# snimu/mixture-of-tokenizers

Measured on AMD Instinct MI355X. Metric: mixed-embed tokens/sec at BxT=256x2048; achieved HBM GB/s vs peak, higher is better.
Workload: dtype f32

## Files before the change

### mixture-of-tokenizers_amd/csrc/mot_embed.hip

```cpp
#include <stdlib.h>

#include <algorithm>

#include "mot_wave.hpp"

namespace mot {

template <int MODE, int NCH, int U, typename T, bool DUAL>
struct MixStream {
    typedef typename Elem<T>::vec vec_t;
    typedef typename Elem<T>::raw raw_t;
    static constexpr int VEC = Elem<T>::kVec;
    const MixArgs &A;
    const WaveLds &W;
    const T *tok_table, *byte_table;
    int lane, Dm, nchunk, ntok;
    int tokv = 0, unit_lane0 = 0;
    bool act[NCH];
    bool tact[NCH];
    raw_t ar[U][NCH];

    __device__ __forceinline__ MixStream(const MixArgs &A_, const WaveLds &W_, int ntok_) : A(A_), W(W_), ntok(ntok_) {
        tok_table = (const T *)A.tok_table;
        byte_table = (const T *)A.byte_table;
// ... 185 lines not shown
#endif
    };
    if (has_ids && A.id_source == MOT_IDS_FROM_TTB) {
        if (A.ttb_elem == 2) {
            if (A.pull_dir == kPullLeft) from_ttb(WaveIndexer<kPullLeft, int16_t>(A, W, row, u0, ntok, dual));
            else if (A.pull_dir == kPullRight) from_ttb(WaveIndexer<kPullRight, int16_t>(A, W, row, u0, ntok, dual));
            else from_ttb(WaveIndexer<kPullNone, int16_t>(A, W, row, u0, ntok, dual));
        } else {
            if (A.pull_dir == kPullLeft) from_ttb(WaveIndexer<kPullLeft, int32_t>(A, W, row, u0, ntok, dual));
            else if (A.pull_dir == kPullRight) from_ttb(WaveIndexer<kPullRight, int32_t>(A, W, row, u0, ntok, dual));
            else from_ttb(WaveIndexer<kPullNone, int32_t>(A, W, row, u0, ntok, dual));
        }
    } else {
        S.tokv = lane < ntok ? A.tokens[row * A.T + u0 + lane] : 0;
        S.request(0);
        if (has_ids) wave_ids_given(A, W, row, u0, ntok);
        else if (A.counters && lane == 0) atomicAdd((unsigned long long *)A.counters, (unsigned long long)ntok);
    }

    T *orow = (T *)A.out + (row * A.T + u0) * (int64_t)S.Dm;
    S.run([&](int t) { return orow + (int64_t)t * S.Dm; });
}

constexpr int kRouteUnits = 8;
constexpr int64_t kRouteMinTokens = 131072;
constexpr int kClaimShards = 64;
constexpr int kClaimStride = 64;

struct RouteWs {
    uint32_t *claim;
    uint8_t *ends;
    uint8_t *offs;
    uint16_t *ids;
    uint16_t *ids2;
};

template <int DIR, typename E>
__global__ __launch_bounds__(kThreads) void route_index_kernel(const MixArgs A, const RouteWs R) {
    extern __shared__ __attribute__((aligned(16))) unsigned char lds_wave[];
    const int lane = threadIdx.x & 63;
    const int wave = __builtin_amdgcn_readfirstlane(threadIdx.x >> 6);
    if (blockIdx.x < 2) R.claim[(blockIdx.x * kThreads + threadIdx.x) * kClaimStride] = 0;
    const int64_t unit_id = (int64_t)blockIdx.x * kWaves + wave;
    if (unit_id >= A.n_units) return;
    const int64_t row = unit_id / A.units_per_row;
    const int64_t u0 = (unit_id - row * A.units_per_row) * A.unit;
    const int ntok = (int)min((int64_t)A.unit, A.T - u0);
    const bool dual = A.add_padded != 0;
    const WaveLds W = wave_lds_carve(lds_wave + (size_t)wave * A.wave_lds, A.unit, A.bpt, dual, DIR != kPullNone ? A.ttb_elem : 0);
    WaveIndexer<DIR, E> ix(A, W, row, u0, ntok, dual);
    const int tok = ix.tokens();
    ix.load_rows();
    ix.finish();

    const int bpt = A.bpt, sv = bpt | 1, n = ntok * bpt;
    const int64_t base = (row * A.T + u0) * bpt;
    for (int i = lane; i < n; i += 64) {
        const int t = i / bpt, k = i - t * bpt;
        R.ids[base + i] = (uint16_t)W.ids[t * sv + k];
        if (dual) R.ids2[base + i] = (uint16_t)W.ids2[t * sv + k];
    }
    const bool in = ix.in_unit;
    const int b = tok & 7;
    int rank = 0, end = 0, acc = 0;
#pragma unroll
    for (int q = 0; q < 8; ++q) {
        const unsigned long long m = __ballot(in && b == q);
        if (in && b == q) rank = acc + (int)__builtin_amdgcn_mbcnt_hi((unsigned)(m >> 32), __builtin_amdgcn_mbcnt_lo((unsigned)m, 0u));
        acc += __popcll(m);
        if (lane == q) end = acc;
    }
    if (in) R.offs[unit_id * A.unit + rank] = (uint8_t)ix.j;
    if (lane < 8) R.ends[unit_id * 8 + lane] = (uint8_t)end;
}

template <int NCH, int U, typename T, bool DUAL>
__global__ __launch_bounds__(kThreads) void embed_mix_routed_kernel(const MixArgs A, const RouteWs R) {
    extern __shared__ __attribute__((aligned(16))) unsigned char lds_wave[];
    const int lane = threadIdx.x & 63;
    const int wave = __builtin_amdgcn_readfirstlane(threadIdx.x >> 6);
    const WaveLds W = wave_lds_carve(lds_wave + (size_t)wave * A.wave_lds, 64, A.bpt, DUAL, 0);
    MixStream<MOT_MIX_SUM, NCH, U, T, DUAL> S(A, W, 0);
    const int bpt = A.bpt, sv = bpt | 1;
    const int64_t n_chunks = (A.n_units + kRouteUnits - 1) / kRouteUnits;
    const int home = blockIdx.x & 7;
    const int shard = ((blockIdx.x >> 3) * kWaves + wave) % kClaimShards;
    for (int q = 0; q < 8;) {
        const int b = (home + q) & 7;
        const int64_t lo = n_chunks * shard / kClaimShards, hi = n_chunks * (shard + 1) / kClaimShards;
        uint32_t k = 0;
        if (lane == 0) k = atomicAdd(R.claim + (b * kClaimShards + shard) * kClaimStride, 1u);
        const int64_t c = lo + __builtin_amdgcn_readfirstlane(k);
        if (c >= hi) { ++q; continue; }
        const int64_t uc = c * kRouteUnits;
        int nb = 0, sb = 0;
        if (lane < kRouteUnits && uc + lane < A.n_units) {
            const uint8_t *e = R.ends + (uc + lane) * 8;
            sb = b ? e[b - 1] : 0;
            nb = e[b] - sb;
        }
        const int incl = wave_scan_add(nb), excl = incl - nb;
        const int total = __builtin_amdgcn_readlane(incl, kRouteUnits - 1);
        for (int p0 = 0; p0 < total; p0 += 64) {
            const int l = p0 + lane;
            int g = 0;
#pragma unroll
            for (int gg = 1; gg < kRouteUnits; ++gg) g = l >= __builtin_amdgcn_readlane(excl, gg) ? gg : g;
            const int ex = __shfl(excl, g, 64), st = __shfl(sb, g, 64);
            int64_t pos = 0;
            int tok = 0;
            if (l < total) {
                const int64_t u = uc + g;
                const int64_t row = u / A.units_per_row;
                pos = row * A.T + (u - row * A.units_per_row) * A.unit + R.offs[u * A.unit + st + (l - ex)];
                tok = A.tokens[pos];
                if ((uint64_t)(uint32_t)tok >= (uint64_t)A.ttb_rows) tok = 0;
            }
            S.tokv = tok;
            S.ntok = min(64, total - p0);
            S.request(0);
            if (l < total) {
                const uint16_t *ia = R.ids + pos * bpt, *ib = R.ids2 + pos * bpt;
                if ((bpt & 7) == 0) {
                    typedef uint16_t u16x8 __attribute__((ext_vector_type(8)));
                    for (int k = 0; k < bpt; k += 8) {
                        const u16x8 va = *(const u16x8 *)(ia + k);
                        u16x8 vb;
                        if (DUAL) vb = *(const u16x8 *)(ib + k);
#pragma unroll
                        for (int e = 0; e < 8; ++e) {
                            W.ids[lane * sv + k + e] = va[e];
                            if (DUAL) W.ids2[lane * sv + k + e] = vb[e];
                        }
                    }
                } else {
                    for (int k = 0; k < bpt; ++k) {
                        W.ids[lane * sv + k] = ia[k];
                        if (DUAL) W.ids2[lane * sv + k] = ib[k];
                    }
                }
            }
            wave_lds_sync();
            const int plo = (int)(uint32_t)pos, phi = (int)(pos >> 32);
            S.run([&](int t) {
                const int64_t p = (int64_t)(((uint64_t)(uint32_t)__builtin_amdgcn_readlane(phi, t) << 32) |
                                            (uint32_t)__builtin_amdgcn_readlane(plo, t));
                return (T *)A.out + p * (int64_t)S.Dm;
            });
            wave_lds_sync();
        }
    }
}

template <typename T>
__global__ __launch_bounds__(kThreads) void rows_rnorm_kernel(const T *__restrict__ table, int64_t rows, int dim,
                                                              float eps, float *__restrict__ out) {
    const int lane = threadIdx.x & 63;
    const int64_t r = (int64_t)blockIdx.x * kWaves + (threadIdx.x >> 6);
    if (r >= rows) return;
    float ss = 0.f;
    for (int j = lane; j < dim; j += 64) {
        const float v = Elem<T>::load1(table + r * dim + j);
        ss += v * v;
    }
    ss = wave_sum(ss);
    if (lane == 0) out[r] = rms_scale(ss, dim, eps);
}

template <int G, typename IdT, typename T>
__global__ __launch_bounds__(kThreads) void gather_rows_kernel(const IdT *__restrict__ ids_a, const IdT *__restrict__ ids_b,
                                                               int64_t n, const T *__restrict__ table, int64_t rows,
                                                               int dim, int rms, float eps, const float *scale,
                                                               T *__restrict__ out, uint32_t *status, int group, int64_t out_ld,
                                                               uint32_t oor_flag) {
// ... 143 lines not shown
                       uint32_t *status, int dtype, hipStream_t stream) {
    if (n == 0) return MOT_OK;
    const unsigned blocks = (unsigned)((n + kWaves - 1) / kWaves);
    if (dtype == MOT_BF16)
        hipLaunchKernelGGL(concat_rows_kernel<__bf16>, dim3(blocks), dim3(kThreads), 0, stream, tokens, ids, n, (const __bf16 *)tok_table, tok_rows, Dt,
                           (const __bf16 *)byte_table, byte_rows, Db, bpt, norm_tok, byte_rnorm, eps, (__bf16 *)u, K, tok_lo, byte_lo, status);
    else
        hipLaunchKernelGGL(concat_rows_kernel<float>, dim3(blocks), dim3(kThreads), 0, stream, tokens, ids, n, (const float *)tok_table, tok_rows, Dt,
                           (const float *)byte_table, byte_rows, Db, bpt, norm_tok, byte_rnorm, eps, (float *)u, K, tok_lo, byte_lo, status);
    return check_launch("concat_rows_kernel");
}

int launch_rows_rnorm(const void *table, int64_t rows, int dim, float eps, float *out, int dtype, hipStream_t stream) {
    const int64_t rb = (rows + kWaves - 1) / kWaves;
    if (dtype == MOT_BF16)
        hipLaunchKernelGGL(rows_rnorm_kernel<__bf16>, dim3((unsigned)rb), dim3(kThreads), 0, stream, (const __bf16 *)table, rows, dim, eps, out);
    else
        hipLaunchKernelGGL(rows_rnorm_kernel<float>, dim3((unsigned)rb), dim3(kThreads), 0, stream, (const float *)table, rows, dim, eps, out);
    return check_launch("rows_rnorm_kernel");
}

static int pick_unit(int64_t n_tokens) { return n_tokens >= 131072 ? 32 : 16; }

static bool sum_routed(const MotEmbedMixDesc &d) {
    return d.mode == MOT_MIX_SUM && d.id_source == MOT_IDS_FROM_TTB && !d.out_ids_padded && !d.out_ids_pulled && d.bpt > 0 &&
           d.byte_rows <= 65536 && d.n_rows * d.tokens_per_row >= kRouteMinTokens && d.dtype == MOT_F32 &&
           (uint64_t)d.tok_rows * d.tok_dim * sizeof(float) <= ((uint64_t)256 << 20);
}

struct MixWorkspace {
    size_t rnorm, claim, ends, offs, ids, ids2, total;
};
static MixWorkspace mix_workspace(const MotEmbedMixDesc &d) {
    auto up = [](size_t x) { return (x + 255) & ~(size_t)255; };
    MixWorkspace w{};
    w.total = (d.mode != MOT_MIX_NOOP && d.norm_byte) ? up((size_t)d.byte_rows * sizeof(float)) : 0;
    if (!sum_routed(d)) return w;
    const int64_t tokens = d.n_rows * d.tokens_per_row;
    const int unit = pick_unit(tokens);
    const int64_t n_units = d.n_rows * ((d.tokens_per_row + unit - 1) / unit);
    const size_t id_bytes = up((size_t)tokens * d.bpt * sizeof(uint16_t));
    w.claim = w.total;
    w.ends = w.claim + (size_t)8 * kClaimShards * kClaimStride * sizeof(uint32_t);
    w.offs = w.ends + up((size_t)n_units * 8);
    w.ids = w.offs + up((size_t)n_units * unit);
    w.ids2 = w.ids + id_bytes;
    w.total = w.ids2 + (d.add_padded ? id_bytes : 0);
    return w;
}

size_t embed_mix_workspace_bytes(const MotEmbedMixDesc &d) {
    if (d.mode == MOT_MIX_CONCAT_LINEAR) return d.dtype == MOT_BF16 ? embed_mix_linear_bf16_workspace_bytes(d) : embed_mix_linear_workspace_bytes(d);
    return mix_workspace(d).total;
}

template <int DIR, typename E>
static void launch_route_index(const MixArgs &A, const RouteWs &R, int64_t blocks, size_t lds, hipStream_t stream) {
    hipLaunchKernelGGL((route_index_kernel<DIR, E>), dim3((unsigned)blocks), dim3(kThreads), lds, stream, A, R);
}

template <int NCH, int U, typename T, bool DUAL>
static int launch_routed(const MixArgs &A, const RouteWs &R, int64_t blocks, size_t lds, hipStream_t stream) {
    if (A.ttb_elem == 2) {
        if (A.pull_dir == kPullLeft) launch_route_index<kPullLeft, int16_t>(A, R, blocks, lds, stream);
        else if (A.pull_dir == kPullRight) launch_route_index<kPullRight, int16_t>(A, R, blocks, lds, stream);
        else launch_route_index<kPullNone, int16_t>(A, R, blocks, lds, stream);
    } else {
        if (A.pull_dir == kPullLeft) launch_route_index<kPullLeft, int32_t>(A, R, blocks, lds, stream);
        else if (A.pull_dir == kPullRight) launch_route_index<kPullRight, int32_t>(A, R, blocks, lds, stream);
        else launch_route_index<kPullNone, int32_t>(A, R, blocks, lds, stream);
    }
    if (int rc = check_launch("route_index_kernel")) return rc;
    MixArgs Ar = A;
    Ar.wave_lds = (int)wave_lds_bytes(64, A.bpt, DUAL, 0);
    const size_t lds_r = (size_t)Ar.wave_lds * kWaves;
    const void *kern = (const void *)embed_mix_routed_kernel<NCH, U, T, DUAL>;
    int dev = 0, cus = 0, per_cu = 0;
    if (hipGetDevice(&dev) != hipSuccess || hipDeviceGetAttribute(&cus, hipDeviceAttributeMultiprocessorCount, dev) != hipSuccess ||
        hipOccupancyMaxActiveBlocksPerMultiprocessor(&per_cu, kern, kThreads, lds_r) != hipSuccess || per_cu < 1)
        return set_error(MOT_EHIP, "embed_mix: no occupancy for embed_mix_routed_kernel");
    const int64_t grid = std::max<int64_t>(((int64_t)cus * per_cu) & ~(int64_t)7, 8 * kClaimShards / kWaves);
    hipLaunchKernelGGL((embed_mix_routed_kernel<NCH, U, T, DUAL>), dim3((unsigned)grid), dim3(kThreads), lds_r, stream, Ar, R);
    return check_launch("embed_mix_routed_kernel");
}

template <int MODE, int NCH, int U, typename T>
static int launch_mix(const MixArgs &A, int64_t blocks, size_t lds, hipStream_t stream, const RouteWs *route) {
    const bool dual = MODE != MOT_MIX_NOOP && (A.id_source == MOT_IDS_FROM_TTB ? A.add_padded != 0 : A.ids_b != nullptr);
    if constexpr (MODE == MOT_MIX_SUM && sizeof(T) == 4) {
        if (route) return dual ? launch_routed<NCH, U, T, true>(A, *route, blocks, lds, stream) : launch_routed<NCH, U, T, false>(A, *route, blocks, lds, stream);
    }
    if (dual)
        hipLaunchKernelGGL((embed_mix_kernel<MODE, NCH, U, T, true>), dim3((unsigned)blocks), dim3(kThreads), lds, stream, A);
    else
        hipLaunchKernelGGL((embed_mix_kernel<MODE, NCH, U, T, false>), dim3((unsigned)blocks), dim3(kThreads), lds, stream, A);
    return check_launch("embed_mix_kernel");
}

template <int MODE>
static int dispatch_nch(const MixArgs &A, int dtype, int64_t blocks, size_t lds, hipStream_t stream, const RouteWs *route = nullptr) {
    const int Dm = MODE == MOT_MIX_CONCAT ? A.Dt + A.bpt * A.Db : A.Dt;
    if (dtype == MOT_BF16) {
        switch ((Dm / 8 + 63) / 64) {
            case 1: return launch_mix<MODE, 1, 4, __bf16>(A, blocks, lds, stream, route);
            case 2: return launch_mix<MODE, 2, 4, __bf16>(A, blocks, lds, stream, route);
            case 3: return launch_mix<MODE, 3, 2, __bf16>(A, blocks, lds, stream, route);
            case 4: return launch_mix<MODE, 4, 2, __bf16>(A, blocks, lds, stream, route);
            default: return set_error(MOT_EUNSUPPORTED, "embed_mix: model_dim %d > 2048 is not built", Dm);
        }
    }
    switch ((Dm / 4 + 63) / 64) {
        case 1: return launch_mix<MODE, 1, 4, float>(A, blocks, lds, stream, route);
        case 2: return launch_mix<MODE, 2, 4, float>(A, blocks, lds, stream, route);
        case 3: return launch_mix<MODE, 3, 2, float>(A, blocks, lds, stream, route);
        case 4: return launch_mix<MODE, 4, 2, float>(A, blocks, lds, stream, route);
        case 5:
        case 6: return launch_mix<MODE, 6, 1, float>(A, blocks, lds, stream, route);
        case 7:
        case 8: return launch_mix<MODE, 8, 1, float>(A, blocks, lds, stream, route);
        default: return set_error(MOT_EUNSUPPORTED, "embed_mix: model_dim %d > 2048 is not built", Dm);
    }
}


template <typename T, int U, int BPT, bool NORMB, int ADD = 0>
__global__ __launch_bounds__(1024) void embed_mean_lds_kernel(const MixArgs A, int slice_cols, int nslices, int64_t tokens_per_part) {
    extern __shared__ __attribute__((aligned(16))) unsigned char lds_raw[];
    T *tab = (T *)lds_raw;
    constexpr int VEC = Elem<T>::kVec;
    typedef typename Elem<T>::vec vec_t;
    const int tid = threadIdx.x, lane = tid & 63, wave = tid >> 6;
    const int slice = blockIdx.x % nslices;
    const int64_t part = blockIdx.x / nslices;
    const int col0 = slice * slice_cols;
    const int D = A.Dt;
    const T *byte_table = (const T *)A.byte_table, *tok_table = (const T *)A.tok_table;
    const int pieces_per_row = slice_cols / VEC;
    for (int64_t q = tid; q < A.byte_rows * pieces_per_row; q += 1024) {
        const int r = (int)(q / pieces_per_row), c = (int)(q - (int64_t)r * pieces_per_row) * VEC;
        *(typename Elem<T>::raw *)(tab + (size_t)r * slice_cols + c) = Elem<T>::load_raw(byte_table + (int64_t)r * D + col0 + c);
    }
    __syncthreads();
// ... 185 lines not shown
    A.units_per_row = (d.tokens_per_row + A.unit - 1) / A.unit;
    A.n_units = d.n_rows * A.units_per_row;
    const int64_t blocks = (A.n_units + kWaves - 1) / kWaves;
    if (blocks > 0x7fffffffLL) return set_error(MOT_EUNSUPPORTED, "embed_mix: too many units");
    const int stream_eb = (has_ids && d.id_source == MOT_IDS_FROM_TTB && d.pull_dir != MOT_PULL_NONE) ? d.ttb_elem_bytes : 0;
    A.wave_lds = (int)wave_lds_bytes(A.unit, has_ids ? d.bpt : 0, dual, stream_eb);
    const size_t lds = (size_t)A.wave_lds * kWaves;

    const MixWorkspace ws = mix_workspace(d);
    if (ws.total && (!d.workspace || d.workspace_bytes < ws.total))
        return set_error(MOT_EWORKSPACE, "embed_mix: needs %zu workspace bytes, got %zu", ws.total, d.workspace_bytes);
    if (d.mode != MOT_MIX_NOOP && d.norm_byte) {
        float *rn = (float *)((unsigned char *)d.workspace + ws.rnorm);
        int rc = launch_rows_rnorm(d.byte_table, d.byte_rows, d.byte_dim, A.eps, rn, d.dtype, stream);
        if (rc) return rc;
        A.byte_rnorm = rn;
    }
    if (const int sc = mean_lds_slice(d)) {
        return d.dtype == MOT_BF16 ? launch_mean_lds<__bf16>(A, d, sc, stream) : launch_mean_lds<float>(A, d, sc, stream);
    }
    switch (d.mode) {
        case MOT_MIX_NOOP: return dispatch_nch<MOT_MIX_NOOP>(A, d.dtype, blocks, lds, stream);
        case MOT_MIX_SUM: {
            if (sum_routed(d) && A.unit == pick_unit(d.n_rows * d.tokens_per_row)) {
                unsigned char *w = (unsigned char *)d.workspace;
                const RouteWs R{(uint32_t *)(w + ws.claim), w + ws.ends, w + ws.offs, (uint16_t *)(w + ws.ids), (uint16_t *)(w + ws.ids2)};
                return dispatch_nch<MOT_MIX_SUM>(A, d.dtype, blocks, lds, stream, &R);
            }
            return dispatch_nch<MOT_MIX_SUM>(A, d.dtype, blocks, lds, stream);
        }
        case MOT_MIX_MEAN: return dispatch_nch<MOT_MIX_MEAN>(A, d.dtype, blocks, lds, stream);
        case MOT_MIX_CONCAT: return dispatch_nch<MOT_MIX_CONCAT>(A, d.dtype, blocks, lds, stream);
        default: return set_error(MOT_EINVAL, "embed_mix: bad mode %d", d.mode);
    }
}

}
```

### mixture-of-tokenizers_amd/csrc/mot_group.hip

```cpp
#include "mot_mix.hpp"

namespace mot {

constexpr int kRankThreads = 512;
__device__ __forceinline__ int lower_bound_u32(const uint32_t *a, int n, uint32_t v) {
    int lo = 0, hi = n;
    while (lo < hi) {
        const int mid = (lo + hi) >> 1;
        if (a[mid] < v) lo = mid + 1; else hi = mid;
    }
    return lo;
}
__global__ __launch_bounds__(kThreads) void zero_i32_kernel(int32_t *__restrict__ p, int64_t n) {
    for (int64_t i = (int64_t)blockIdx.x * kThreads + threadIdx.x; i < n; i += (int64_t)gridDim.x * kThreads) p[i] = 0;
}

int launch_zero_words(void *p, int64_t n_words, hipStream_t stream) {
    if (n_words <= 0) return MOT_OK;
    int64_t blocks = (n_words + kThreads - 1) / kThreads;
    if (blocks > 2048) blocks = 2048;
    hipLaunchKernelGGL(zero_i32_kernel, dim3((unsigned)blocks), dim3(kThreads), 0, stream, (int32_t *)p, n_words);
    return check_launch("zero_i32_kernel");
}

template <int kRankChunk>
__global__ __launch_bounds__(kRankThreads) void bwd_rank_kernel(const int32_t *__restrict__ tokens, int64_t n, int64_t rows,
                                                                int32_t *__restrict__ counts, int32_t *__restrict__ rank,
                                                                uint32_t *status) {
    __shared__ uint32_t skey[kRankChunk];
    __shared__ int32_t runbase[kRankChunk];
    const int tid = threadIdx.x;
    const int64_t base = (int64_t)blockIdx.x * kRankChunk;
    for (int i = tid; i < kRankChunk; i += kRankThreads) {
        uint32_t key = 0xffffffffu;
        if (base + i < n) {
            uint32_t t = (uint32_t)tokens[base + i];
            if ((uint64_t)t >= (uint64_t)rows) { if (status) atomicOr(status, kStatusTokenOor); t = 0; }
            key = (t << 11) | (uint32_t)i;
        }
        skey[i] = key;
    }
    __syncthreads();
    for (int k = 2; k <= kRankChunk; k <<= 1)
        for (int j = k >> 1; j > 0; j >>= 1) {
            for (int p = tid; p < kRankChunk / 2; p += kRankThreads) {
                const int i = ((p & ~(j - 1)) << 1) | (p & (j - 1)), ixj = i | j;
                const uint32_t x = skey[i], y = skey[ixj];
                if ((x > y) == ((i & k) == 0)) { skey[i] = y; skey[ixj] = x; }
            }
            __syncthreads();
        }
    constexpr int kPer = kRankChunk / kRankThreads;
    int head[kPer];
#pragma unroll
    for (int r = 0; r < kPer; ++r) {
        const int si = tid + r * kRankThreads;
        const uint32_t key = skey[si];
        head[r] = -1;
        if (key == 0xffffffffu) continue;
        const uint32_t tok = key >> 11;
        const int h = (si == 0 || (skey[si - 1] >> 11) != tok) ? si : lower_bound_u32(skey, si, tok << 11);
        head[r] = h;
        if (h == si) {
            const int e = lower_bound_u32(skey, kRankChunk, (tok + 1) << 11);
            runbase[si] = atomicAdd(&counts[tok], e - si);
        }
    }
    __syncthreads();
#pragma unroll
    for (int r = 0; r < kPer; ++r) {
        const int si = tid + r * kRankThreads;
        if (head[r] < 0) continue;
        rank[base + (skey[si] & 2047)] = runbase[head[r]] + (si - head[r]);
    }
}

__global__ __launch_bounds__(kThreads) void bwd_place_kernel(const int32_t *__restrict__ tokens, int64_t n, int64_t rows,
                                                             const int32_t *__restrict__ starts, const int32_t *__restrict__ rank,
                                                             int32_t *__restrict__ pos_sorted, int32_t *__restrict__ tok_sorted) {
    for (int64_t i = (int64_t)blockIdx.x * kThreads + threadIdx.x; i < n; i += (int64_t)gridDim.x * kThreads) {
        int t = tokens[i];
        if ((uint64_t)(uint32_t)t >= (uint64_t)rows) t = 0;
        const int32_t at = starts[t] + rank[i];
        pos_sorted[at] = (int32_t)i;
        tok_sorted[at] = t;
    }
}

__global__ __launch_bounds__(1024) void bwd_scan_kernel(const int32_t *__restrict__ counts, int64_t rows,
                                                        int32_t *__restrict__ starts) {
    __shared__ int32_t wsum[16];
    const int tid = threadIdx.x, lane = tid & 63, wave = tid >> 6;
    const int64_t t0 = (int64_t)blockIdx.x * 1024;
    int32_t before = 0;
    for (int64_t i = tid; i < t0; i += 1024) before += counts[i];
    const int64_t i = t0 + tid;
    const int32_t own = i < rows ? counts[i] : 0;
    const int32_t incl = wave_incl_add(own, lane);
    const int32_t bsum = wave_incl_add(before, lane);
    if (lane == 63) wsum[wave] = incl + bsum;
    __syncthreads();
    int32_t off = incl - own;
    for (int w = 0; w < 16; ++w) off += w < wave ? wsum[w] : 0;
    __shared__ int32_t bpart[16];
    if (lane == 63) bpart[wave] = bsum;
    __syncthreads();
    for (int w = wave; w < 16; ++w) off += bpart[w];
    if (i < rows) starts[i] = off;
}

size_t group_positions_ws_ints(int64_t n, int64_t rows) { return 2 * (size_t)rows + 3 * (size_t)n; }
int launch_group_positions(const int32_t *ids, int64_t n, int64_t rows, int32_t *ws_ints, const int32_t **pos_sorted_out, const int32_t **id_sorted_out,
                           uint32_t *status, hipStream_t stream) {
    if (rows >= (1 << 21) - 1) return set_error(MOT_EUNSUPPORTED, "group_positions: %lld rows (>= 2^21 - 1) are not built", (long long)rows);
    int32_t *counts = ws_ints, *starts = counts + rows, *rank = starts + rows, *pos_sorted = rank + n, *id_sorted = pos_sorted + n;
    int rc;
    if ((rc = launch_zero_words(counts, rows, stream))) return rc;
    const int rank_chunk = n >= 256 * 2048 ? 2048 : 512;
    const int64_t rb = (n + rank_chunk - 1) / rank_chunk;
    int64_t pb = (n + kThreads - 1) / kThreads;
    if (pb > 2048) pb = 2048;
    if (rb > 0x7fffffffLL) return set_error(MOT_EUNSUPPORTED, "group_positions: too many positions");
    if (n > 0) {
        if (rank_chunk == 2048)
            hipLaunchKernelGGL(bwd_rank_kernel<2048>, dim3((unsigned)rb), dim3(kRankThreads), 0, stream, ids, n, rows, counts, rank, status);
        else
            hipLaunchKernelGGL(bwd_rank_kernel<512>, dim3((unsigned)rb), dim3(kRankThreads), 0, stream, ids, n, rows, counts, rank, status);
        hipLaunchKernelGGL(bwd_scan_kernel, dim3((unsigned)((rows + 1023) / 1024)), dim3(1024), 0, stream, counts, rows, starts);
        hipLaunchKernelGGL(bwd_place_kernel, dim3((unsigned)pb), dim3(kThreads), 0, stream, ids, n, rows, starts, rank, pos_sorted, id_sorted);
        if ((rc = check_launch("group_positions kernels"))) return rc;
    }
    *pos_sorted_out = pos_sorted;
    *id_sorted_out = id_sorted;
    return MOT_OK;
}

}
```

### mixture-of-tokenizers_amd/csrc/mot_internal.hpp

```cpp
#pragma once
#include <hip/hip_runtime.h>
#include <stdint.h>

#include <atomic>

#include "../../include/mot.h"

namespace mot {

int set_error(int code, const char *fmt, ...) __attribute__((format(printf, 2, 3)));
int check_launch(const char *what);

int ensure_max_dyn_lds(const void *kernel, std::atomic<uint64_t> &done, const char *name);

int pick_tile_tokens(int64_t n_rows, int64_t tokens_per_row, int bpt, bool with_ids);

int launch_tokens_to_bytes(const int32_t *tokens, int64_t n_tokens, const void *ttb, int elem, int64_t ttb_rows,
                           int bpt, int64_t *out, uint32_t *status, hipStream_t stream);
int launch_pull_bytes(const int64_t *in, int64_t *out, int64_t B, int64_t tokens_per_row, int bpt, int64_t pad,
                      int64_t eot, int dir, hipStream_t stream);
int launch_create_batch(const int32_t *tokens, int64_t B, int64_t T, const void *ttb_left, const void *ttb_right,
                        int elem, int64_t ttb_rows, int bpt, int32_t pad, int32_t eot, int64_t *out, uint32_t *status,
                        hipStream_t stream);
int launch_char_matrix(const int32_t *codes, const int64_t *tok_off, const int64_t *seq_off, int64_t n_seqs, int64_t seq_len, int max_char,
// ... 28 lines not shown
size_t embed_mix_linear_composed_workspace_bytes(const MotEmbedMixDesc &d);
int launch_embed_mix_linear_composed(const MotEmbedMixDesc &d, hipStream_t stream);
bool concat16_usable(const MotEmbedMixDesc &d);
bool concat16_norm_in_kernel(const MotEmbedMixDesc &d);
bool concat16_residual_usable(const MotEmbedMixDesc &d);
int launch_concat16(const MotEmbedMixDesc &d, const int32_t *tokens, const int64_t *ids, const uint16_t *ids16, int64_t n, const float *rn_byte,
                    void *out, float *row_rnorm, hipStream_t stream, bool residual = false);
int launch_wave_ids16(const MotEmbedMixDesc &d, uint16_t *ids16, hipStream_t stream);
int launch_gemm_rows_bf16(const void *A, int lda, int64_t n, const void *B, int ldb, int R, int Nc, void *C, int ldc, bool out_bf16,
                          const void *bias, hipStream_t stream, bool accumulate = false, const float *addend = nullptr);
bool gemm_rows_bf16_256_usable(const void *A, int lda, int64_t n, const void *B, int ldb, int R, int Nc);
bool gemm_rows_f32_256_usable(const float *A, int lda, int64_t n, const float *B, int ldb, int R, int Nc);
int launch_gemm_rows_f32_256(const float *A, int lda, int64_t n, const float *B, int ldb, int R, int Nc, float *C, int ldc, const float *bias, bool accumulate,
                             hipStream_t stream);
int launch_gemm_tn_bf16(const __bf16 *A, int lda, int M, const __bf16 *B, int ldb, int Kc, int64_t rows, float *C, int ldc, hipStream_t stream);
int launch_transpose_f32(const float *src, int rows, int cols, float *dst, hipStream_t stream);
int launch_widen(const void *src_bf16, size_t n, float *dst, hipStream_t stream);
int launch_narrow(const float *src, int64_t n, void *dst_bf16, hipStream_t stream);
int launch_transpose_bf16(const void *src_bf16, int rows, int cols, void *dst_bf16, hipStream_t stream);
int launch_narrow_transpose(const float *src, int rows, int cols, void *dst_bf16, hipStream_t stream);
size_t group_positions_ws_ints(int64_t n, int64_t rows);
int launch_group_positions(const int32_t *ids, int64_t n, int64_t rows, int32_t *ws_ints, const int32_t **pos_sorted, const int32_t **id_sorted,
                           uint32_t *status, hipStream_t stream);
int launch_zero_words(void *p, int64_t n_words, hipStream_t stream);
size_t cross_attn_bwd_workspace_bytes(const MotCrossAttnDesc &d);
int launch_cross_attn_bwd(const MotCrossAttnDesc &d, const MotCrossAttnGrads &g, hipStream_t stream);
size_t char_swa_workspace_bytes(const MotCharSwaDesc &d);
int launch_char_swa(const MotCharSwaDesc &d, hipStream_t stream);
size_t cross_attn_workspace_bytes(const MotCrossAttnDesc &d);
int launch_cross_attn(const MotCrossAttnDesc &d, hipStream_t stream);
int byte_head_check(const MotByteHeadDesc *d);
size_t byte_head_workspace_bytes(const MotByteHeadDesc &d);
int launch_byte_head_fwd(const MotByteHeadDesc &d, hipStream_t stream);
int launch_byte_head_bwd(const MotByteHeadDesc &d, const float *grad_loss, void *dx, float *dW, hipStream_t stream);
size_t byte_self_attn_saved_bytes(const MotByteSelfAttnDesc &d);
size_t byte_self_attn_workspace_bytes(const MotByteSelfAttnDesc &d);
int launch_byte_self_attn_fwd(const MotByteSelfAttnDesc &d, hipStream_t stream);
int launch_byte_self_attn_bwd(const MotByteSelfAttnDesc &d, const MotByteSelfAttnGrads &g, hipStream_t stream);
int byte_fc_check(const MotByteFcMixDesc *d, const MotByteFcMixGrads *g, bool backward);
size_t byte_fc_mix_workspace_bytes(const MotByteFcMixDesc *d);
size_t byte_fc_mix_bwd_workspace_bytes(const MotByteFcMixDesc *d);
int launch_byte_fc_mix_fwd(const MotByteFcMixDesc &d, hipStream_t stream);
int launch_byte_fc_mix_bwd(const MotByteFcMixDesc &d, const MotByteFcMixGrads &g, hipStream_t stream);

}
```

Before: 1.288 billion.

## Replace claim-based bucket routing with full token-id grouping sort for sum mix

The routed sum path used per-unit 8-way buckets on token low bits and an atomic claim scheduler. It is replaced with a global counting sort of positions by token id, reusing the backward group_positions machinery. The rank phase is fused into the index kernel as extra leading blocks. The gather kernel then processes sorted 64-token runs so repeated token rows are fetched close together. This aims at better L2 reuse of the token table and drops the dynamic claiming, but it adds zeroing, scan and place kernel launches plus extra workspace traffic.

```diff
diff --git a/mixture-of-tokenizers_amd/csrc/mot_embed.hip b/mixture-of-tokenizers_amd/csrc/mot_embed.hip
--- a/mixture-of-tokenizers_amd/csrc/mot_embed.hip
+++ b/mixture-of-tokenizers_amd/csrc/mot_embed.hip
@@ -231,26 +231,30 @@
     S.run([&](int t) { return orow + (int64_t)t * S.Dm; });
 }
 
-constexpr int kRouteUnits = 8;
-constexpr int64_t kRouteMinTokens = 131072;
-constexpr int kClaimShards = 64;
-constexpr int kClaimStride = 64;
-
-struct RouteWs {
-    uint32_t *claim;
-    uint8_t *ends;
-    uint8_t *offs;
+constexpr int64_t kGroupMinTokens = 131072;
+
+struct GroupWs {
     uint16_t *ids;
     uint16_t *ids2;
+    const int32_t *pos_sorted, *id_sorted;
+    int64_t n;
+    int64_t rows;
+    int32_t *counts, *rank;
+    int rank_blocks;
 };
+constexpr int kGroupRankChunk = 512;
 
 template <int DIR, typename E>
-__global__ __launch_bounds__(kThreads) void route_index_kernel(const MixArgs A, const RouteWs R) {
+__global__ __launch_bounds__(kThreads) void group_index_kernel(const MixArgs A, const GroupWs G) {
     extern __shared__ __attribute__((aligned(16))) unsigned char lds_wave[];
     const int lane = threadIdx.x & 63;
     const int wave = __builtin_amdgcn_readfirstlane(threadIdx.x >> 6);
-    if (blockIdx.x < 2) R.claim[(blockIdx.x * kThreads + threadIdx.x) * kClaimStride] = 0;
-    const int64_t unit_id = (int64_t)blockIdx.x * kWaves + wave;
+    if ((int)blockIdx.x < G.rank_blocks) {
+        rank_positions_block<kGroupRankChunk, kThreads>(A.tokens, G.n, G.rows, G.counts, G.rank, A.status, kStatusTokenOor, blockIdx.x,
+                                                        (uint32_t *)lds_wave, (int32_t *)lds_wave + kGroupRankChunk);
+        return;
+    }
+    const int64_t unit_id = (int64_t)((int)blockIdx.x - G.rank_blocks) * kWaves + wave;
     if (unit_id >= A.n_units) return;
     const int64_t row = unit_id / A.units_per_row;
     const int64_t u0 = (unit_id - row * A.units_per_row) * A.unit;
@@ -258,7 +262,7 @@
     const bool dual = A.add_padded != 0;
     const WaveLds W = wave_lds_carve(lds_wave + (size_t)wave * A.wave_lds, A.unit, A.bpt, dual, DIR != kPullNone ? A.ttb_elem : 0);
     WaveIndexer<DIR, E> ix(A, W, row, u0, ntok, dual);
-    const int tok = ix.tokens();
+    ix.tokens();
     ix.load_rows();
     ix.finish();
 
@@ -266,99 +270,53 @@
     const int64_t base = (row * A.T + u0) * bpt;
     for (int i = lane; i < n; i += 64) {
         const int t = i / bpt, k = i - t * bpt;
-        R.ids[base + i] = (uint16_t)W.ids[t * sv + k];
-        if (dual) R.ids2[base + i] = (uint16_t)W.ids2[t * sv + k];
-    }
-    const bool in = ix.in_unit;
-    const int b = tok & 7;
-    int rank = 0, end = 0, acc = 0;
-#pragma unroll
-    for (int q = 0; q < 8; ++q) {
-        const unsigned long long m = __ballot(in && b == q);
-        if (in && b == q) rank = acc + (int)__builtin_amdgcn_mbcnt_hi((unsigned)(m >> 32), __builtin_amdgcn_mbcnt_lo((unsigned)m, 0u));
-        acc += __popcll(m);
-        if (lane == q) end = acc;
-    }
-    if (in) R.offs[unit_id * A.unit + rank] = (uint8_t)ix.j;
-    if (lane < 8) R.ends[unit_id * 8 + lane] = (uint8_t)end;
+        G.ids[base + i] = (uint16_t)W.ids[t * sv + k];
+        if (dual) G.ids2[base + i] = (uint16_t)W.ids2[t * sv + k];
+    }
 }
 
 template <int NCH, int U, typename T, bool DUAL>
-__global__ __launch_bounds__(kThreads) void embed_mix_routed_kernel(const MixArgs A, const RouteWs R) {
+__global__ __launch_bounds__(kThreads) void embed_mix_grouped_kernel(const MixArgs A, const GroupWs G) {
     extern __shared__ __attribute__((aligned(16))) unsigned char lds_wave[];
     const int lane = threadIdx.x & 63;
     const int wave = __builtin_amdgcn_readfirstlane(threadIdx.x >> 6);
+    const int64_t s0 = ((int64_t)blockIdx.x * kWaves + wave) * 64;
+    if (s0 >= G.n) return;
+    const int ntok = (int)min((int64_t)64, G.n - s0);
     const WaveLds W = wave_lds_carve(lds_wave + (size_t)wave * A.wave_lds, 64, A.bpt, DUAL, 0);
-    MixStream<MOT_MIX_SUM, NCH, U, T, DUAL> S(A, W, 0);
+    MixStream<MOT_MIX_SUM, NCH, U, T, DUAL> S(A, W, ntok);
     const int bpt = A.bpt, sv = bpt | 1;
-    const int64_t n_chunks = (A.n_units + kRouteUnits - 1) / kRouteUnits;
-    const int home = blockIdx.x & 7;
-    const int shard = ((blockIdx.x >> 3) * kWaves + wave) % kClaimShards;
-    for (int q = 0; q < 8;) {
-        const int b = (home + q) & 7;
-        const int64_t lo = n_chunks * shard / kClaimShards, hi = n_chunks * (shard + 1) / kClaimShards;
-        uint32_t k = 0;
-        if (lane == 0) k = atomicAdd(R.claim + (b * kClaimShards + shard) * kClaimStride, 1u);
-        const int64_t c = lo + __builtin_amdgcn_readfirstlane(k);
-        if (c >= hi) { ++q; continue; }
-        const int64_t uc = c * kRouteUnits;
-        int nb = 0, sb = 0;
-        if (lane < kRouteUnits && uc + lane < A.n_units) {
-            const uint8_t *e = R.ends + (uc + lane) * 8;
-            sb = b ? e[b - 1] : 0;
-            nb = e[b] - sb;
-        }
-        const int incl = wave_scan_add(nb), excl = incl - nb;
-        const int total = __builtin_amdgcn_readlane(incl, kRouteUnits - 1);
-        for (int p0 = 0; p0 < total; p0 += 64) {
-            const int l = p0 + lane;
-            int g = 0;
-#pragma unroll
-            for (int gg = 1; gg < kRouteUnits; ++gg) g = l >= __builtin_amdgcn_readlane(excl, gg) ? gg : g;
-            const int ex = __shfl(excl, g, 64), st = __shfl(sb, g, 64);
-            int64_t pos = 0;
-            int tok = 0;
-            if (l < total) {
-                const int64_t u = uc + g;
-                const int64_t row = u / A.units_per_row;
-                pos = row * A.T + (u - row * A.units_per_row) * A.unit + R.offs[u * A.unit + st + (l - ex)];
-                tok = A.tokens[pos];
-                if ((uint64_t)(uint32_t)tok >= (uint64_t)A.ttb_rows) tok = 0;
-            }
-            S.tokv = tok;
-            S.ntok = min(64, total - p0);
-            S.request(0);
-            if (l < total) {
-                const uint16_t *ia = R.ids + pos * bpt, *ib = R.ids2 + pos * bpt;
-                if ((bpt & 7) == 0) {
-                    typedef uint16_t u16x8 __attribute__((ext_vector_type(8)));
-                    for (int k = 0; k < bpt; k += 8) {
-                        const u16x8 va = *(const u16x8 *)(ia + k);
-                        u16x8 vb;
-                        if (DUAL) vb = *(const u16x8 *)(ib + k);
-#pragma unroll
-                        for (int e = 0; e < 8; ++e) {
-                            W.ids[lane * sv + k + e] = va[e];
-                            if (DUAL) W.ids2[lane * sv + k + e] = vb[e];
-                        }
-                    }
-                } else {
-                    for (int k = 0; k < bpt; ++k) {
-                        W.ids[lane * sv + k] = ia[k];
-                        if (DUAL) W.ids2[lane * sv + k] = ib[k];
-                    }
-                }
-            }
-            wave_lds_sync();
-            const int plo = (int)(uint32_t)pos, phi = (int)(pos >> 32);
-            S.run([&](int t) {
-                const int64_t p = (int64_t)(((uint64_t)(uint32_t)__builtin_amdgcn_readlane(phi, t) << 32) |
-                                            (uint32_t)__builtin_amdgcn_readlane(plo, t));
-                return (T *)A.out + p * (int64_t)S.Dm;
-            });
-            wave_lds_sync();
-        }
-    }
+    int pos = 0, tok = 0;
+    if (lane < ntok) {
+        pos = G.pos_sorted[s0 + lane];
+        tok = G.id_sorted[s0 + lane];
+    }
+    S.tokv = tok;
+    S.unit_lane0 = 0;
+    S.request(0);
+    if (lane < ntok) {
+        const uint16_t *ia = G.ids + (int64_t)pos * bpt, *ib = G.ids2 + (int64_t)pos * bpt;
+        if ((bpt & 7) == 0) {
+            typedef uint16_t u16x8 __attribute__((ext_vector_type(8)));
+            for (int k = 0; k < bpt; k += 8) {
+                const u16x8 va = *(const u16x8 *)(ia + k);
+                u16x8 vb;
+                if (DUAL) vb = *(const u16x8 *)(ib + k);
+#pragma unroll
+                for (int e = 0; e < 8; ++e) {
+                    W.ids[lane * sv + k + e] = va[e];
+                    if (DUAL) W.ids2[lane * sv + k + e] = vb[e];
+                }
+            }
+        } else {
+            for (int k = 0; k < bpt; ++k) {
+                W.ids[lane * sv + k] = ia[k];
+                if (DUAL) W.ids2[lane * sv + k] = ib[k];
+            }
+        }
+    }
+    wave_lds_sync();
+    S.run([&](int t) { return (T *)A.out + (int64_t)__builtin_amdgcn_readlane(pos, t) * S.Dm; });
 }
 
 template <typename T>
@@ -548,30 +506,27 @@
 
 static int pick_unit(int64_t n_tokens) { return n_tokens >= 131072 ? 32 : 16; }
 
-static bool sum_routed(const MotEmbedMixDesc &d) {
+static bool sum_grouped(const MotEmbedMixDesc &d) {
     return d.mode == MOT_MIX_SUM && d.id_source == MOT_IDS_FROM_TTB && !d.out_ids_padded && !d.out_ids_pulled && d.bpt > 0 &&
-           d.byte_rows <= 65536 && d.n_rows * d.tokens_per_row >= kRouteMinTokens && d.dtype == MOT_F32 &&
-           (uint64_t)d.tok_rows * d.tok_dim * sizeof(float) <= ((uint64_t)256 << 20);
-}
+           d.byte_rows <= 65536 && d.n_rows * d.tokens_per_row >= kGroupMinTokens && d.n_rows * d.tokens_per_row <= 0x7fffffffLL &&
+           d.tok_rows < (1 << 21) - 1 && d.dtype == MOT_F32;
+}
+static int64_t group_rows(const MotEmbedMixDesc &d) { return std::min(d.tok_rows, d.ttb_rows); }
 
 struct MixWorkspace {
-    size_t rnorm, claim, ends, offs, ids, ids2, total;
+    size_t rnorm, ids, ids2, group, total;
 };
 static MixWorkspace mix_workspace(const MotEmbedMixDesc &d) {
     auto up = [](size_t x) { return (x + 255) & ~(size_t)255; };
     MixWorkspace w{};
     w.total = (d.mode != MOT_MIX_NOOP && d.norm_byte) ? up((size_t)d.byte_rows * sizeof(float)) : 0;
-    if (!sum_routed(d)) return w;
+    if (!sum_grouped(d)) return w;
     const int64_t tokens = d.n_rows * d.tokens_per_row;
-    const int unit = pick_unit(tokens);
-    const int64_t n_units = d.n_rows * ((d.tokens_per_row + unit - 1) / unit);
     const size_t id_bytes = up((size_t)tokens * d.bpt * sizeof(uint16_t));
-    w.claim = w.total;
-    w.ends = w.claim + (size_t)8 * kClaimShards * kClaimStride * sizeof(uint32_t);
-    w.offs = w.ends + up((size_t)n_units * 8);
-    w.ids = w.offs + up((size_t)n_units * unit);
+    w.ids = w.total;
     w.ids2 = w.ids + id_bytes;
-    w.total = w.ids2 + (d.add_padded ? id_bytes : 0);
+    w.group = w.ids2 + (d.add_padded ? id_bytes : 0);
+    w.total = w.group + up(group_positions_ws_ints(tokens, group_rows(d)) * sizeof(int32_t));
     return w;
 }
 
@@ -581,40 +536,42 @@
 }
 
 template <int DIR, typename E>
-static void launch_route_index(const MixArgs &A, const RouteWs &R, int64_t blocks, size_t lds, hipStream_t stream) {
-    hipLaunchKernelGGL((route_index_kernel<DIR, E>), dim3((unsigned)blocks), dim3(kThreads), lds, stream, A, R);
+static void launch_group_index(const MixArgs &A, const GroupWs &G, int64_t blocks, size_t lds, hipStream_t stream) {
+    hipLaunchKernelGGL((group_index_kernel<DIR, E>), dim3((unsigned)blocks), dim3(kThreads), lds, stream, A, G);
 }
 
 template <int NCH, int U, typename T, bool DUAL>
-static int launch_routed(const MixArgs &A, const RouteWs &R, int64_t blocks, size_t lds, hipStream_t stream) {
+static int launch_grouped(const MixArgs &A, GroupWs G, int32_t *sort_ws, int64_t blocks, size_t lds, hipStream_t stream) {
+    GroupParts parts;
+    if (int rc = group_positions_begin(G.n, G.rows, sort_ws, &parts, stream)) return rc;
+    G.counts = parts.counts; G.rank = parts.rank; G.pos_sorted = parts.pos_sorted; G.id_sorted = parts.id_sorted;
+    G.rank_blocks = (int)((G.n + kGroupRankChunk - 1) / kGroupRankChunk);
+    blocks += G.rank_blocks;
+    if (blocks > 0x7fffffffLL) return set_error(MOT_EUNSUPPORTED, "embed_mix: too many units");
+    lds = std::max(lds, (size_t)2 * kGroupRankChunk * sizeof(int32_t));
     if (A.ttb_elem == 2) {
-        if (A.pull_dir == kPullLeft) launch_route_index<kPullLeft, int16_t>(A, R, blocks, lds, stream);
-        else if (A.pull_dir == kPullRight) launch_route_index<kPullRight, int16_t>(A, R, blocks, lds, stream);
-        else launch_route_index<kPullNone, int16_t>(A, R, blocks, lds, stream);
+        if (A.pull_dir == kPullLeft) launch_group_index<kPullLeft, int16_t>(A, G, blocks, lds, stream);
+        else if (A.pull_dir == kPullRight) launch_group_index<kPullRight, int16_t>(A, G, blocks, lds, stream);
+        else launch_group_index<kPullNone, int16_t>(A, G, blocks, lds, stream);
     } else {
-        if (A.pull_dir == kPullLeft) launch_route_index<kPullLeft, int32_t>(A, R, blocks, lds, stream);
-        else if (A.pull_dir == kPullRight) launch_route_index<kPullRight, int32_t>(A, R, blocks, lds, stream);
-        else launch_route_index<kPullNone, int32_t>(A, R, blocks, lds, stream);
-    }
-    if (int rc = check_launch("route_index_kernel")) return rc;
-    MixArgs Ar = A;
-    Ar.wave_lds = (int)wave_lds_bytes(64, A.bpt, DUAL, 0);
-    const size_t lds_r = (size_t)Ar.wave_lds * kWaves;
-    const void *kern = (const void *)embed_mix_routed_kernel<NCH, U, T, DUAL>;
-    int dev = 0, cus = 0, per_cu = 0;
-    if (hipGetDevice(&dev) != hipSuccess || hipDeviceGetAttribute(&cus, hipDeviceAttributeMultiprocessorCount, dev) != hipSuccess ||
-        hipOccupancyMaxActiveBlocksPerMultiprocessor(&per_cu, kern, kThreads, lds_r) != hipSuccess || per_cu < 1)
-        return set_error(MOT_EHIP, "embed_mix: no occupancy for embed_mix_routed_kernel");
-    const int64_t grid = std::max<int64_t>(((int64_t)cus * per_cu) & ~(int64_t)7, 8 * kClaimShards / kWaves);
-    hipLaunchKernelGGL((embed_mix_routed_kernel<NCH, U, T, DUAL>), dim3((unsigned)grid), dim3(kThreads), lds_r, stream, Ar, R);
-    return check_launch("embed_mix_routed_kernel");
+        if (A.pull_dir == kPullLeft) launch_group_index<kPullLeft, int32_t>(A, G, blocks, lds, stream);
+        else if (A.pull_dir == kPullRight) launch_group_index<kPullRight, int32_t>(A, G, blocks, lds, stream);
+        else launch_group_index<kPullNone, int32_t>(A, G, blocks, lds, stream);
+    }
+    if (int rc = check_launch("group_index_kernel")) return rc;
+    if (int rc = group_positions_finish(A.tokens, G.n, G.rows, parts, stream)) return rc;
+    MixArgs Ag = A;
+    Ag.wave_lds = (int)wave_lds_bytes(64, A.bpt, DUAL, 0);
+    const int64_t grid = (G.n + 64 * kWaves - 1) / (64 * kWaves);
+    hipLaunchKernelGGL((embed_mix_grouped_kernel<NCH, U, T, DUAL>), dim3((unsigned)grid), dim3(kThreads), (size_t)Ag.wave_lds * kWaves, stream, Ag, G);
+    return check_launch("embed_mix_grouped_kernel");
 }
 
 template <int MODE, int NCH, int U, typename T>
-static int launch_mix(const MixArgs &A, int64_t blocks, size_t lds, hipStream_t stream, const RouteWs *route) {
+static int launch_mix(const MixArgs &A, int64_t blocks, size_t lds, hipStream_t stream, const GroupWs *group, int32_t *sort_ws) {
     const bool dual = MODE != MOT_MIX_NOOP && (A.id_source == MOT_IDS_FROM_TTB ? A.add_padded != 0 : A.ids_b != nullptr);
     if constexpr (MODE == MOT_MIX_SUM && sizeof(T) == 4) {
-        if (route) return dual ? launch_routed<NCH, U, T, true>(A, *route, blocks, lds, stream) : launch_routed<NCH, U, T, false>(A, *route, blocks, lds, stream);
+        if (group) return dual ? launch_grouped<NCH, U, T, true>(A, *group, sort_ws, blocks, lds, stream) : launch_grouped<NCH, U, T, false>(A, *group, sort_ws, blocks, lds, stream);
     }
     if (dual)
         hipLaunchKernelGGL((embed_mix_kernel<MODE, NCH, U, T, true>), dim3((unsigned)blocks), dim3(kThreads), lds, stream, A);
@@ -624,26 +581,26 @@
 }
 
 template <int MODE>
-static int dispatch_nch(const MixArgs &A, int dtype, int64_t blocks, size_t lds, hipStream_t stream, const RouteWs *route = nullptr) {
+static int dispatch_nch(const MixArgs &A, int dtype, int64_t blocks, size_t lds, hipStream_t stream, const GroupWs *group = nullptr, int32_t *sort_ws = nullptr) {
     const int Dm = MODE == MOT_MIX_CONCAT ? A.Dt + A.bpt * A.Db : A.Dt;
     if (dtype == MOT_BF16) {
         switch ((Dm / 8 + 63) / 64) {
-            case 1: return launch_mix<MODE, 1, 4, __bf16>(A, blocks, lds, stream, route);
-            case 2: return launch_mix<MODE, 2, 4, __bf16>(A, blocks, lds, stream, route);
-            case 3: return launch_mix<MODE, 3, 2, __bf16>(A, blocks, lds, stream, route);
-            case 4: return launch_mix<MODE, 4, 2, __bf16>(A, blocks, lds, stream, route);
+            case 1: return launch_mix<MODE, 1, 4, __bf16>(A, blocks, lds, stream, group, sort_ws);
+            case 2: return launch_mix<MODE, 2, 4, __bf16>(A, blocks, lds, stream, group, sort_ws);
+            case 3: return launch_mix<MODE, 3, 2, __bf16>(A, blocks, lds, stream, group, sort_ws);
+            case 4: return launch_mix<MODE, 4, 2, __bf16>(A, blocks, lds, stream, group, sort_ws);
             default: return set_error(MOT_EUNSUPPORTED, "embed_mix: model_dim %d > 2048 is not built", Dm);
         }
     }
     switch ((Dm / 4 + 63) / 64) {
-        case 1: return launch_mix<MODE, 1, 4, float>(A, blocks, lds, stream, route);
-        case 2: return launch_mix<MODE, 2, 4, float>(A, blocks, lds, stream, route);
-        case 3: return launch_mix<MODE, 3, 2, float>(A, blocks, lds, stream, route);
-        case 4: return launch_mix<MODE, 4, 2, float>(A, blocks, lds, stream, route);
+        case 1: return launch_mix<MODE, 1, 4, float>(A, blocks, lds, stream, group, sort_ws);
+        case 2: return launch_mix<MODE, 2, 4, float>(A, blocks, lds, stream, group, sort_ws);
+        case 3: return launch_mix<MODE, 3, 2, float>(A, blocks, lds, stream, group, sort_ws);
+        case 4: return launch_mix<MODE, 4, 2, float>(A, blocks, lds, stream, group, sort_ws);
         case 5:
-        case 6: return launch_mix<MODE, 6, 1, float>(A, blocks, lds, stream, route);
+        case 6: return launch_mix<MODE, 6, 1, float>(A, blocks, lds, stream, group, sort_ws);
         case 7:
-        case 8: return launch_mix<MODE, 8, 1, float>(A, blocks, lds, stream, route);
+        case 8: return launch_mix<MODE, 8, 1, float>(A, blocks, lds, stream, group, sort_ws);
         default: return set_error(MOT_EUNSUPPORTED, "embed_mix: model_dim %d > 2048 is not built", Dm);
     }
 }
@@ -875,10 +832,12 @@
     switch (d.mode) {
         case MOT_MIX_NOOP: return dispatch_nch<MOT_MIX_NOOP>(A, d.dtype, blocks, lds, stream);
         case MOT_MIX_SUM: {
-            if (sum_routed(d) && A.unit == pick_unit(d.n_rows * d.tokens_per_row)) {
+            if (sum_grouped(d) && A.unit == pick_unit(d.n_rows * d.tokens_per_row)) {
                 unsigned char *w = (unsigned char *)d.workspace;
-                const RouteWs R{(uint32_t *)(w + ws.claim), w + ws.ends, w + ws.offs, (uint16_t *)(w + ws.ids), (uint16_t *)(w + ws.ids2)};
-                return dispatch_nch<MOT_MIX_SUM>(A, d.dtype, blocks, lds, stream, &R);
+                GroupWs G{};
+                G.ids = (uint16_t *)(w + ws.ids); G.ids2 = (uint16_t *)(w + ws.ids2);
+                G.n = d.n_rows * d.tokens_per_row; G.rows = group_rows(d);
+                return dispatch_nch<MOT_MIX_SUM>(A, d.dtype, blocks, lds, stream, &G, (int32_t *)(w + ws.group));
             }
             return dispatch_nch<MOT_MIX_SUM>(A, d.dtype, blocks, lds, stream);
         }
diff --git a/mixture-of-tokenizers_amd/csrc/mot_group.hip b/mixture-of-tokenizers_amd/csrc/mot_group.hip
--- a/mixture-of-tokenizers_amd/csrc/mot_group.hip
+++ b/mixture-of-tokenizers_amd/csrc/mot_group.hip
@@ -3,14 +3,6 @@
 namespace mot {
 
 constexpr int kRankThreads = 512;
-__device__ __forceinline__ int lower_bound_u32(const uint32_t *a, int n, uint32_t v) {
-    int lo = 0, hi = n;
-    while (lo < hi) {
-        const int mid = (lo + hi) >> 1;
-        if (a[mid] < v) lo = mid + 1; else hi = mid;
-    }
-    return lo;
-}
 __global__ __launch_bounds__(kThreads) void zero_i32_kernel(int32_t *__restrict__ p, int64_t n) {
     for (int64_t i = (int64_t)blockIdx.x * kThreads + threadIdx.x; i < n; i += (int64_t)gridDim.x * kThreads) p[i] = 0;
 }
@@ -29,50 +21,7 @@
                                                                 uint32_t *status) {
     __shared__ uint32_t skey[kRankChunk];
     __shared__ int32_t runbase[kRankChunk];
-    const int tid = threadIdx.x;
-    const int64_t base = (int64_t)blockIdx.x * kRankChunk;
-    for (int i = tid; i < kRankChunk; i += kRankThreads) {
-        uint32_t key = 0xffffffffu;
-        if (base + i < n) {
-            uint32_t t = (uint32_t)tokens[base + i];
-            if ((uint64_t)t >= (uint64_t)rows) { if (status) atomicOr(status, kStatusTokenOor); t = 0; }
-            key = (t << 11) | (uint32_t)i;
-        }
-        skey[i] = key;
-    }
-    __syncthreads();
-    for (int k = 2; k <= kRankChunk; k <<= 1)
-        for (int j = k >> 1; j > 0; j >>= 1) {
-            for (int p = tid; p < kRankChunk / 2; p += kRankThreads) {
-                const int i = ((p & ~(j - 1)) << 1) | (p & (j - 1)), ixj = i | j;
-                const uint32_t x = skey[i], y = skey[ixj];
-                if ((x > y) == ((i & k) == 0)) { skey[i] = y; skey[ixj] = x; }
-            }
-            __syncthreads();
-        }
-    constexpr int kPer = kRankChunk / kRankThreads;
-    int head[kPer];
-#pragma unroll
-    for (int r = 0; r < kPer; ++r) {
-        const int si = tid + r * kRankThreads;
-        const uint32_t key = skey[si];
-        head[r] = -1;
-        if (key == 0xffffffffu) continue;
-        const uint32_t tok = key >> 11;
-        const int h = (si == 0 || (skey[si - 1] >> 11) != tok) ? si : lower_bound_u32(skey, si, tok << 11);
-        head[r] = h;
-        if (h == si) {
-            const int e = lower_bound_u32(skey, kRankChunk, (tok + 1) << 11);
-            runbase[si] = atomicAdd(&counts[tok], e - si);
-        }
-    }
-    __syncthreads();
-#pragma unroll
-    for (int r = 0; r < kPer; ++r) {
-        const int si = tid + r * kRankThreads;
-        if (head[r] < 0) continue;
-        rank[base + (skey[si] & 2047)] = runbase[head[r]] + (si - head[r]);
-    }
+    rank_positions_block<kRankChunk, kRankThreads>(tokens, n, rows, counts, rank, status, kStatusTokenOor, blockIdx.x, skey, runbase);
 }
 
 __global__ __launch_bounds__(kThreads) void bwd_place_kernel(const int32_t *__restrict__ tokens, int64_t n, int64_t rows,
@@ -110,28 +59,36 @@
 }
 
 size_t group_positions_ws_ints(int64_t n, int64_t rows) { return 2 * (size_t)rows + 3 * (size_t)n; }
+int group_positions_begin(int64_t n, int64_t rows, int32_t *ws_ints, GroupParts *p, hipStream_t stream) {
+    if (rows >= (1 << 21) - 1) return set_error(MOT_EUNSUPPORTED, "group_positions: %lld rows (>= 2^21 - 1) are not built", (long long)rows);
+    if ((n + 511) / 512 > 0x7fffffffLL) return set_error(MOT_EUNSUPPORTED, "group_positions: too many positions");
+    p->counts = ws_ints; p->starts = p->counts + rows; p->rank = p->starts + rows; p->pos_sorted = p->rank + n; p->id_sorted = p->pos_sorted + n;
+    return launch_zero_words(p->counts, rows, stream);
+}
+int group_positions_finish(const int32_t *ids, int64_t n, int64_t rows, const GroupParts &p, hipStream_t stream) {
+    if (n <= 0) return MOT_OK;
+    int64_t pb = (n + kThreads - 1) / kThreads;
+    if (pb > 2048) pb = 2048;
+    hipLaunchKernelGGL(bwd_scan_kernel, dim3((unsigned)((rows + 1023) / 1024)), dim3(1024), 0, stream, p.counts, rows, p.starts);
+    hipLaunchKernelGGL(bwd_place_kernel, dim3((unsigned)pb), dim3(kThreads), 0, stream, ids, n, rows, p.starts, p.rank, p.pos_sorted, p.id_sorted);
+    return check_launch("group_positions kernels");
+}
 int launch_group_positions(const int32_t *ids, int64_t n, int64_t rows, int32_t *ws_ints, const int32_t **pos_sorted_out, const int32_t **id_sorted_out,
                            uint32_t *status, hipStream_t stream) {
-    if (rows >= (1 << 21) - 1) return set_error(MOT_EUNSUPPORTED, "group_positions: %lld rows (>= 2^21 - 1) are not built", (long long)rows);
-    int32_t *counts = ws_ints, *starts = counts + rows, *rank = starts + rows, *pos_sorted = rank + n, *id_sorted = pos_sorted + n;
+    GroupParts p;
     int rc;
-    if ((rc = launch_zero_words(counts, rows, stream))) return rc;
+    if ((rc = group_positions_begin(n, rows, ws_ints, &p, stream))) return rc;
     const int rank_chunk = n >= 256 * 2048 ? 2048 : 512;
     const int64_t rb = (n + rank_chunk - 1) / rank_chunk;
-    int64_t pb = (n + kThreads - 1) / kThreads;
-    if (pb > 2048) pb = 2048;
-    if (rb > 0x7fffffffLL) return set_error(MOT_EUNSUPPORTED, "group_positions: too many positions");
     if (n > 0) {
         if (rank_chunk == 2048)
-            hipLaunchKernelGGL(bwd_rank_kernel<2048>, dim3((unsigned)rb), dim3(kRankThreads), 0, stream, ids, n, rows, counts, rank, status);
+            hipLaunchKernelGGL(bwd_rank_kernel<2048>, dim3((unsigned)rb), dim3(kRankThreads), 0, stream, ids, n, rows, p.counts, p.rank, status);
         else
-            hipLaunchKernelGGL(bwd_rank_kernel<512>, dim3((unsigned)rb), dim3(kRankThreads), 0, stream, ids, n, rows, counts, rank, status);
-        hipLaunchKernelGGL(bwd_scan_kernel, dim3((unsigned)((rows + 1023) / 1024)), dim3(1024), 0, stream, counts, rows, starts);
-        hipLaunchKernelGGL(bwd_place_kernel, dim3((unsigned)pb), dim3(kThreads), 0, stream, ids, n, rows, starts, rank, pos_sorted, id_sorted);
-        if ((rc = check_launch("group_positions kernels"))) return rc;
+            hipLaunchKernelGGL(bwd_rank_kernel<512>, dim3((unsigned)rb), dim3(kRankThreads), 0, stream, ids, n, rows, p.counts, p.rank, status);
+        if ((rc = group_positions_finish(ids, n, rows, p, stream))) return rc;
     }
-    *pos_sorted_out = pos_sorted;
-    *id_sorted_out = id_sorted;
+    *pos_sorted_out = p.pos_sorted;
+    *id_sorted_out = p.id_sorted;
     return MOT_OK;
 }
 
diff --git a/mixture-of-tokenizers_amd/csrc/mot_internal.hpp b/mixture-of-tokenizers_amd/csrc/mot_internal.hpp
--- a/mixture-of-tokenizers_amd/csrc/mot_internal.hpp
+++ b/mixture-of-tokenizers_amd/csrc/mot_internal.hpp
@@ -74,6 +74,11 @@
 size_t group_positions_ws_ints(int64_t n, int64_t rows);
 int launch_group_positions(const int32_t *ids, int64_t n, int64_t rows, int32_t *ws_ints, const int32_t **pos_sorted, const int32_t **id_sorted,
                            uint32_t *status, hipStream_t stream);
+struct GroupParts {
+    int32_t *counts, *starts, *rank, *pos_sorted, *id_sorted;
+};
+int group_positions_begin(int64_t n, int64_t rows, int32_t *ws_ints, GroupParts *p, hipStream_t stream);
+int group_positions_finish(const int32_t *ids, int64_t n, int64_t rows, const GroupParts &p, hipStream_t stream);
 int launch_zero_words(void *p, int64_t n_words, hipStream_t stream);
 size_t cross_attn_bwd_workspace_bytes(const MotCrossAttnDesc &d);
 int launch_cross_attn_bwd(const MotCrossAttnDesc &d, const MotCrossAttnGrads &g, hipStream_t stream);
@@ -95,4 +100,62 @@
 int launch_byte_fc_mix_fwd(const MotByteFcMixDesc &d, hipStream_t stream);
 int launch_byte_fc_mix_bwd(const MotByteFcMixDesc &d, const MotByteFcMixGrads &g, hipStream_t stream);
 
+__device__ __forceinline__ int lower_bound_u32(const uint32_t *a, int n, uint32_t v) {
+    int lo = 0, hi = n;
+    while (lo < hi) {
+        const int mid = (lo + hi) >> 1;
+        if (a[mid] < v) lo = mid + 1; else hi = mid;
+    }
+    return lo;
 }
+template <int kChunk, int kThr>
+__device__ __forceinline__ void rank_positions_block(const int32_t *__restrict__ tokens, int64_t n, int64_t rows, int32_t *__restrict__ counts,
+                                                     int32_t *__restrict__ rank, uint32_t *status, uint32_t oor_flag, int64_t block,
+                                                     uint32_t *skey, int32_t *runbase) {
+    const int tid = threadIdx.x;
+    const int64_t base = block * kChunk;
+    for (int i = tid; i < kChunk; i += kThr) {
+        uint32_t key = 0xffffffffu;
+        if (base + i < n) {
+            uint32_t t = (uint32_t)tokens[base + i];
+            if ((uint64_t)t >= (uint64_t)rows) { if (status) atomicOr(status, oor_flag); t = 0; }
+            key = (t << 11) | (uint32_t)i;
+        }
+        skey[i] = key;
+    }
+    __syncthreads();
+    for (int k = 2; k <= kChunk; k <<= 1)
+        for (int j = k >> 1; j > 0; j >>= 1) {
+            for (int p = tid; p < kChunk / 2; p += kThr) {
+                const int i = ((p & ~(j - 1)) << 1) | (p & (j - 1)), ixj = i | j;
+                const uint32_t x = skey[i], y = skey[ixj];
+                if ((x > y) == ((i & k) == 0)) { skey[i] = y; skey[ixj] = x; }
+            }
+            __syncthreads();
+        }
+    constexpr int kPer = kChunk / kThr;
+    int head[kPer];
+#pragma unroll
+    for (int r = 0; r < kPer; ++r) {
+        const int si = tid + r * kThr;
+        const uint32_t key = skey[si];
+        head[r] = -1;
+        if (key == 0xffffffffu) continue;
+        const uint32_t tok = key >> 11;
+        const int h = (si == 0 || (skey[si - 1] >> 11) != tok) ? si : lower_bound_u32(skey, si, tok << 11);
+        head[r] = h;
+        if (h == si) {
+            const int e = lower_bound_u32(skey, kChunk, (tok + 1) << 11);
+            runbase[si] = atomicAdd(&counts[tok], e - si);
+        }
+    }
+    __syncthreads();
+#pragma unroll
+    for (int r = 0; r < kPer; ++r) {
+        const int si = tid + r * kThr;
+        if (head[r] < 0) continue;
+        rank[base + (skey[si] & 2047)] = runbase[head[r]] + (si - head[r]);
+    }
+}
+
+}
```

Measured after the change: 1.298 billion (median of 6 runs). About the same (+0.7%).
